# coreyjadams/SparseEventID

Measured on NVIDIA B200. Metric: 3D sparse ResNet train events/sec, higher is better.
Workload: dtype bf16

## Files before the change

sparseeventid_b200/csrc/conv_tc.cu:

```cuda
#include <cstdlib>
#include <cstring>

#include "common.cuh"
#include "tc_ptx.cuh"

namespace tc {

constexpr int BM = 128;
constexpr int KC = 64;
constexpr int KC_TF32 = 32;
constexpr int A_BYTES = BM * 128;
constexpr int EPI_WARPS = 4;
constexpr int NGRP = 4;
constexpr int PROD_WARPS = 4 * NGRP;
constexpr int WARP_MMA = EPI_WARPS + PROD_WARPS;
constexpr int MMA_WARPS = 4;
constexpr int WARP_BLOAD = WARP_MMA + MMA_WARPS;
constexpr int THREADS = 32 * (WARP_BLOAD + 1);
constexpr int MAX_A = 12, MAX_B = 8;
constexpr int MASK_BYTES = 32;
constexpr int LIST_BYTES = 64 * 8;
using namespace tcptx;

__device__ __forceinline__ uint64_t make_desc_sw128(uint32_t saddr) {
  uint64_t d = 0;
  d |= (uint64_t)((saddr & 0x3FFFFu) >> 4);
  d |= (uint64_t)1 << 16;
  d |= (uint64_t)(1024 >> 4) << 32;
  d |= (uint64_t)1 << 46;
  d |= (uint64_t)2 << 61;
  return d;
}
__device__ __forceinline__ const unsigned char* mad_wide16(uint32_t units, const unsigned char* base) {
  uint64_t r;
  asm("mad.wide.u32 %0, %1, 16, %2;" : "=l"(r) : "r"(units), "l"((uint64_t)(uintptr_t)base));
  return reinterpret_cast<const unsigned char*>((uintptr_t)r);
}
template <bool TF32>
__device__ __forceinline__ uint32_t make_idesc(int n) {
  constexpr uint32_t fmt = TF32 ? 2u : 1u;
  return (1u << 4) | (fmt << 7) | (fmt << 10) | ((uint32_t)(n >> 3) << 17) | ((uint32_t)(BM >> 4) << 24);
}
template <bool TF32>
__device__ __forceinline__ void store8(void* out, int64_t idx, const float* f) {
  if constexpr (TF32) {
    float4* d = reinterpret_cast<float4*>(reinterpret_cast<float*>(out) + idx);
    d[0] = make_float4(f[0], f[1], f[2], f[3]);
    d[1] = make_float4(f[4], f[5], f[6], f[7]);
  } else {
    uint4 u;
    u.x = pack_bf16x2(f[0], f[1]); u.y = pack_bf16x2(f[2], f[3]);
    u.z = pack_bf16x2(f[4], f[5]); u.w = pack_bf16x2(f[6], f[7]);
    *reinterpret_cast<uint4*>(reinterpret_cast<__nv_bfloat16*>(out) + idx) = u;
  }
}
struct Params {
  const void* in;
  const int32_t* nbr;
  const unsigned char* bimg;
  const float* bias;
  void* out;
  int64_t n_rows, n_pad;
  int K, n_in, n_out;
  int nch;
  int last_kc;
  int T;
  int SA, SB;
  int num_tiles;
  int NM;
  int nbuf;
  int ksplit;
  unsigned long long* dbg;
  int exp;
};

template <int NCH, bool PAIR, bool TF32 = false>
__global__ void __launch_bounds__(THREADS, 1) k_conv_tc(const Params p) {
  static_assert(!(TF32 && PAIR), "a 32-channel fp32 row fills a stage");
  constexpr int ESZ = TF32 ? 4 : 2;
  constexpr int KCE = 128 / ESZ;
  const int nch = NCH > 0 ? NCH : p.nch;
  extern __shared__ unsigned char smem_raw[];
  pdl_launch_dependents();
  const uint32_t raw = smem_u32(smem_raw);
  const uint32_t base = (raw + 1023u) & ~1023u;
  unsigned char* gbase = smem_raw + (base - raw);
  const int SA = p.SA, SB = p.SB;
  const uint32_t b_bytes = (uint32_t)p.n_out * 128u;
  const uint32_t a_base = base;
  const uint32_t b_base = base + (uint32_t)SA * A_BYTES;
  const uint32_t bar0 = b_base + (uint32_t)SB * b_bytes;
  auto afull = [&](int s) { return bar0 + 8u * (uint32_t)s; };
  auto aempty = [&](int s) { return bar0 + 8u * (uint32_t)(MAX_A + s); };
  auto bfull = [&](int s) { return bar0 + 8u * (uint32_t)(2 * MAX_A + s); };
  auto bempty = [&](int s) { return bar0 + 8u * (uint32_t)(2 * MAX_A + MAX_B + s); };
  auto accf = [&](int b) { return bar0 + 8u * (uint32_t)(2 * MAX_A + 2 * MAX_B + b); };
  auto acce = [&](int b) { return bar0 + 8u * (uint32_t)(2 * MAX_A + 2 * MAX_B + 2 + b); };
  constexpr int NBAR = 2 * MAX_A + 2 * MAX_B + 4;
  unsigned char* tail = gbase + (size_t)SA * A_BYTES + (size_t)SB * b_bytes + 8 * NBAR;
  uint32_t* tmem_slot = reinterpret_cast<uint32_t*>(tail);
  uint32_t* amask = reinterpret_cast<uint32_t*>(tail + 16);
  unsigned char* lists = tail + 16 + MAX_A * MASK_BYTES;

  const int warp = __shfl_sync(0xffffffffu, (int)(threadIdx.x >> 5), 0), lane = threadIdx.x & 31;
  auto mark = [&](int role, int stage, int ev) {
#ifdef SCN_TC_TIMELINE
    if (p.dbg != nullptr && blockIdx.x == 0 && lane == 0 && stage < 256)
      p.dbg[((size_t)role * 256 + stage) * 8 + ev] = (unsigned long long)clock64();
#else
    (void)role; (void)stage; (void)ev;
#endif
  };
#ifdef SCN_TC_TIMELINE
  const int exp_flags = p.exp;
#else
  constexpr int exp_flags = 0;
#endif

  const int T = p.T;
  const int tile_lo = (int)(((int64_t)p.num_tiles * blockIdx.x) / gridDim.x);
  const int tile_hi = (int)(((int64_t)p.num_tiles * (blockIdx.x + 1)) / gridDim.x);
  const int my_tiles = tile_hi - tile_lo;
  const int my_groups = (my_tiles + T - 1) / T;
  auto tiles_in_group = [&](int g) { return my_tiles - g * T < T ? my_tiles - g * T : T; };
  const int NSTEP = PAIR ? (p.K + 1) / 2 : p.K;
  const int Q = NSTEP * nch;
  const bool ksplit = p.ksplit != 0 && p.NM == 2 && my_tiles == 1;

  if (warp == WARP_MMA) {
    if (lane == 0) {
      for (int s = 0; s < SA; ++s) {
        mbar_init(afull(s), 132);
        mbar_init(aempty(s), 1);
      }
      for (int s = 0; s < SB; ++s) {
        mbar_init(bfull(s), 1);
        mbar_init(bempty(s), ksplit ? 1 : p.NM);
      }
      for (int b = 0; b < 2; ++b) {
        mbar_init(accf(b), p.NM);
        mbar_init(acce(b), EPI_WARPS);
      }
      asm volatile("fence.mbarrier_init.release.cluster;" ::: "memory");
    }
    __syncwarp();
    asm volatile("tcgen05.alloc.cta_group::1.sync.aligned.shared::cta.b32 [%0], %1;" ::"r"(smem_u32(tmem_slot)), "r"(512)
                 : "memory");
    asm volatile("tcgen05.relinquish_alloc_permit.cta_group::1.sync.aligned;" ::: "memory");
  }
  tc_fence_before();
  __syncthreads();
  tc_fence_after();
  const uint32_t tmem_base = *tmem_slot;
  pdl_wait();

  const int NM = p.NM;
  const int spc = SA / NM;

  if (warp >= EPI_WARPS && warp < EPI_WARPS + PROD_WARPS) {
    const int pw = warp - EPI_WARPS;
    const int grp = pw >> 2, wq = pw & 3;
    const int cls = grp % NM, sub = grp / NM, gpc = NGRP / NM;
    constexpr int LPI = PAIR ? 4 : 8;
    constexpr int IPP = 32 / LPI;
    const int chunk = lane % LPI, isub = lane / LPI;
    const uint32_t row_vec = (uint32_t)p.n_in >> (TF32 ? 2 : 3);
    const int last_chunks = p.last_kc * ESZ / 16;
    const uint32_t lt = (1u << lane) - 1u;
    const uint32_t csw = (uint32_t)chunk << 4;
    const uint32_t myrow = 32u * (uint32_t)wq + (uint32_t)lane;
    const uint32_t drow = a_base + (myrow << 7) + ((myrow & 7u) << 4);

    int t = cls, q = 0, cc = 0, g = 0, tv = my_groups > 0 ? tiles_in_group(0) : 0;
    const int32_t* gptr = p.nbr + (int64_t)tile_lo * BM + myrow;
    const int32_t* qptr = gptr;
    const int64_t qstride = (int64_t)p.n_pad * (PAIR ? 2 : 1);
    auto next_q = [&]() {
      ++q;
      if (++cc == nch) { cc = 0; qptr += qstride; }
    };
    auto step = [&]() {
      if (ksplit) {
        next_q(); next_q();
        if (q >= Q) { g = my_groups; tv = 0; }
        return;
      }
      t += NM;
      if (t >= tv) {
        t = cls;
        next_q();
        if (q == Q) {
          q = 0; ++g;
          gptr += (int64_t)T * BM;
          qptr = gptr;
          tv = g < my_groups ? tiles_in_group(g) : 0;
        }
      }
    };
    auto valid = [&]() { return g < my_groups && (ksplit ? q < Q : cls < tv); };
    if (ksplit) {
      t = 0;
      if (cls == 1) next_q();
    }
    for (int i = 0; i < sub; ++i)
      if (valid()) step();
    auto fetch = [&](int& jl_, int& jh_, int& q_) {
      q_ = -1; jl_ = -1; jh_ = -1;
      if (valid()) {
        const int32_t* src = qptr + t * BM;
        jl_ = ldg_nc32(src);
        if (PAIR && (2 * q + 1 < p.K)) jh_ = ldg_nc32(src + p.n_pad);
        q_ = (q << 3) | cc;
        for (int i = 0; i < gpc; ++i) step();
      }
    };

    int ls = sub;
    uint32_t round = 0;
    int it = 0;
    auto do_stage = [&](const int jl, const int jh, const int qc) {
      if (wq == 0) mark(grp, it, 0);
      int2* list = reinterpret_cast<int2*>(lists + (pw * 2 + (it & 1)) * LIST_BYTES);
      const int slot = cls * spc + ls;
      const int ccur = qc & 7;
      const bool full = qc < (ksplit ? 16 : 8);
      const uint32_t dst = drow + (uint32_t)slot * A_BYTES;
      const uint32_t bl = __ballot_sync(0xffffffffu, jl >= 0);
      const uint32_t bh = PAIR ? __ballot_sync(0xffffffffu, jh >= 0) : 0u;
      int nlive;
      if (full) {
        list[lane] = make_int2(jl >= 0 ? (int)((uint32_t)jl * row_vec) : -1, (int)dst);
        if (PAIR) list[32 + lane] = make_int2(jh >= 0 ? (int)((uint32_t)jh * row_vec) : -1, (int)(dst ^ 0x40u));
        nlive = PAIR ? 64 : 32;
      } else {
        const int2 el = make_int2((int)((uint32_t)jl * row_vec), (int)dst);
        const int2 eh = make_int2((int)((uint32_t)jh * row_vec), (int)(dst ^ 0x40u));
        if (jl >= 0) list[__popc(bl & lt)] = el;
        nlive = __popc(bl);
        if (PAIR) {
          if (jh >= 0) list[nlive + __popc(bh & lt)] = eh;
          nlive += __popc(bh);
        }
        if (nlive & (IPP - 1)) {
          const bool from_hi = PAIR && bh != 0u;
          const int top = 31 - __clz(from_hi ? bh : bl);
          const int lx = __shfl_sync(0xffffffffu, from_hi ? eh.x : el.x, top);
          const int ly = __shfl_sync(0xffffffffu, from_hi ? eh.y : el.y, top);
          const int padded = (nlive + IPP - 1) & ~(IPP - 1);
          if (nlive + lane < padded) list[nlive + lane] = make_int2(lx, ly);
        }
      }
      __syncwarp();
      if (wq == 0) mark(grp, it, 1);

      mbar_wait(aempty(slot), (round & 1u) ^ 1u);
      if (wq == 0) mark(grp, it, 2);
      if (lane == 0) {
        amask[slot * 8 + wq] = ~bl;
        if (PAIR) amask[slot * 8 + 4 + wq] = ~bh;
      }
      const int npass = (nlive + IPP - 1) / IPP;
      const bool lane_on = PAIR ? true : chunk < (ccur == nch - 1 ? last_chunks : 8);
      const unsigned char* src0 = reinterpret_cast<const unsigned char*>(p.in) + ((uint32_t)ccur * 128u + csw);
      if (lane_on && !(exp_flags & 1)) {
        if (!full) {
          for (int p0 = 0; p0 < npass; p0 += 4) {
            int2 e[4];
#pragma unroll
            for (int u = 0; u < 4; ++u)
              if (p0 + u < npass) e[u] = list[(p0 + u) * IPP + isub];
#pragma unroll
            for (int u = 0; u < 4; ++u)
              if (p0 + u < npass) cp_async16((uint32_t)e[u].y ^ csw, mad_wide16((uint32_t)e[u].x, src0), 16u);
          }
        } else {
#pragma unroll
          for (int pass = 0; pass < 8; ++pass) {
            const int2 e = list[pass * IPP + isub];
            const bool live = e.x != -1;
            cp_async16((uint32_t)e.y ^ csw, mad_wide16(live ? (uint32_t)e.x : 0u, src0), live ? 16u : 0u);
          }
        }
      }
      cp_async_arrive_noinc(afull(slot));
      if (lane == 0) mbar_arrive(afull(slot));
      if (wq == 0) mark(grp, it, 3);
      ++it;
      ls += gpc;
      if (ls >= spc) { ls -= spc; ++round; }
    };

    int jlA, jhA, qA, jlB, jhB, qB;
    fetch(jlA, jhA, qA);
    fetch(jlB, jhB, qB);
    while (qA >= 0) {
      int jlC, jhC, qC;
      fetch(jlC, jhC, qC);
      do_stage(jlA, jhA, qA);
      jlA = jlB; jhA = jhB; qA = qB;
      jlB = jlC; jhB = jhC; qB = qC;
    }
  } else if (warp == WARP_BLOAD) {
    const int total_b = my_groups * Q;
    int bslot = 0;
    uint32_t bround = 0;
    for (int i = 0; i < total_b; ++i) {
      mark(8, i, 0);
      if (ksplit) mbar_wait_sleep(bempty(bslot), (bround & 1u) ^ 1u, 100u);
      else mbar_wait(bempty(bslot), (bround & 1u) ^ 1u);
      mark(8, i, 1);
      if (elect_one()) {
        mbar_expect_tx(bfull(bslot), b_bytes);
        bulk_g2s(b_base + (uint32_t)bslot * b_bytes, p.bimg + (size_t)(i % Q) * b_bytes, b_bytes, bfull(bslot));
      }
      __syncwarp();
      if (++bslot == SB) { bslot = 0; ++bround; }
    }
  } else if (warp >= WARP_MMA && warp < WARP_MMA + MMA_WARPS) {
    const int m = warp - WARP_MMA;
    if (m < NM) {
      const uint32_t idesc = make_idesc<TF32>(p.n_out);
      const uint64_t da0 = make_desc_sw128(a_base), db0 = make_desc_sw128(b_base);
      const int nbuf = p.nbuf;
      int bslot = 0;
      uint32_t bround = 0;
      int ls = 0;
      uint32_t around = 0;
      int it = 0;
      auto issue_stage = [&](int q, uint32_t col, uint64_t db, bool first) {
        const int cc = PAIR ? 0 : q % nch;
        const int step = PAIR ? q : q / nch;
        const int nk = PAIR ? ((2 * step + 1 < p.K) ? 4 : 2) : ((cc == nch - 1 ? p.last_kc : KCE) * ESZ / 32);
        const int aslot = m * spc + ls;
        mark(4 + m, it, 0);
        mbar_wait(afull(aslot), around & 1u);
        mark(4 + m, it, 1);
        tc_fence_after();
        uint32_t m0 = 0, m1 = 0, m2 = 0, m3 = 0, h0 = 0, h1 = 0, h2 = 0, h3 = 0;
        if (!first) {
          const uint4 mw = *reinterpret_cast<const uint4*>(amask + aslot * 8);
          m0 = __ballot_sync(0xffffffffu, (mw.x >> lane) & 1u);
          m1 = __ballot_sync(0xffffffffu, (mw.y >> lane) & 1u);
          m2 = __ballot_sync(0xffffffffu, (mw.z >> lane) & 1u);
          m3 = __ballot_sync(0xffffffffu, (mw.w >> lane) & 1u);
          if (PAIR) {
            const uint4 hw = *reinterpret_cast<const uint4*>(amask + aslot * 8 + 4);
            h0 = __ballot_sync(0xffffffffu, (hw.x >> lane) & 1u);
            h1 = __ballot_sync(0xffffffffu, (hw.y >> lane) & 1u);
            h2 = __ballot_sync(0xffffffffu, (hw.z >> lane) & 1u);
            h3 = __ballot_sync(0xffffffffu, (hw.w >> lane) & 1u);
          }
        }
        const uint64_t da = da0 + (uint64_t)((uint32_t)aslot * (A_BYTES >> 4));
        const uint32_t tmem_d = tmem_base + col;
        if (elect_one()) {
#pragma unroll
          for (int kk = 0; kk < 4; ++kk) {
            if (kk < nk && !(exp_flags & 2)) {
              const bool hi = PAIR && kk >= 2;
              umma_masked<TF32>(tmem_d, da + (uint64_t)(kk * 2), db + (uint64_t)(kk * 2), idesc, (!first || kk > 0) ? 1u : 0u,
                                hi ? h0 : m0, hi ? h1 : m1, hi ? h2 : m2, hi ? h3 : m3);
            }
          }
          umma_commit(aempty(aslot));
        }
        __syncwarp();
        mark(4 + m, it, 2);
        ++it;
        if (++ls == spc) { ls = 0; ++around; }
      };
      if (ksplit) {
        mbar_wait(acce(0), 1u);
        tc_fence_after();
        bslot = m;
        for (int q = m; q < Q; q += 2) {
          mbar_wait(bfull(bslot), bround & 1u);
          issue_stage(q, (uint32_t)(m * p.n_out), db0 + (uint64_t)(((uint32_t)bslot * b_bytes) >> 4), q < 2);
          if (elect_one()) umma_commit(bempty(bslot));
          __syncwarp();
          bslot += 2;
          if (bslot >= SB) { bslot -= SB; ++bround; }
        }
        if (elect_one()) umma_commit(accf(0));
        __syncwarp();
      } else
      for (int g = 0; g < my_groups; ++g) {
        const int buf = nbuf == 2 ? (g & 1) : 0;
        const uint32_t use = (uint32_t)(nbuf == 2 ? (g >> 1) : g);
        const int tv = tiles_in_group(g);
        mbar_wait(acce(buf), (use & 1u) ^ 1u);
        tc_fence_after();
        for (int q = 0; q < Q; ++q) {
          mark(10 + m, g * Q + q, 0);
          mbar_wait(bfull(bslot), bround & 1u);
          mark(10 + m, g * Q + q, 1);
          const uint64_t db = db0 + (uint64_t)(((uint32_t)bslot * b_bytes) >> 4);
          for (int t = m; t < tv; t += NM) issue_stage(q, (uint32_t)buf * 256u + (uint32_t)(t * p.n_out), db, q == 0);
          if (elect_one()) umma_commit(bempty(bslot));
          __syncwarp();
          if (++bslot == SB) { bslot = 0; ++bround; }
        }
        if (elect_one()) umma_commit(accf(buf));
        __syncwarp();
      }
    }
  } else if (warp < EPI_WARPS) {
    if (ksplit) {
      mbar_wait_sleep(accf(0), 0u, 100u);
      tc_fence_after();
      const int64_t row = (int64_t)tile_lo * BM + warp * 32 + lane;
      const uint32_t taddr = tmem_base + ((uint32_t)(warp * 32) << 16);
      for (int c0 = 0; c0 < p.n_out; c0 += 16) {
        uint32_t a[16], b[16];
        tmem_ld16x2(taddr + (uint32_t)c0, taddr + (uint32_t)(p.n_out + c0), a, b);
        if (row < p.n_rows && !(exp_flags & 4)) {
#pragma unroll
          for (int gq = 0; gq < 2; ++gq) {
            float f[8];
#pragma unroll
            for (int e = 0; e < 8; ++e)
              f[e] = __uint_as_float(a[gq * 8 + e]) + __uint_as_float(b[gq * 8 + e]) +
                     (p.bias ? __ldg(p.bias + c0 + gq * 8 + e) : 0.f);
            store8<TF32>(p.out, row * p.n_out + c0 + gq * 8, f);
          }
        }
      }
      tc_fence_before();
    } else
    for (int g = 0; g < my_groups; ++g) {
      const int buf = p.nbuf == 2 ? (g & 1) : 0;
      if (warp == 0) mark(9, g, 0);
      mbar_wait_long(accf(buf), (uint32_t)(p.nbuf == 2 ? (g >> 1) : g) & 1u);
      if (warp == 0) mark(9, g, 1);
      tc_fence_after();
      const int tv = tiles_in_group(g);
      for (int t = 0; t < tv; ++t) {
        const int64_t tile = (int64_t)tile_lo + (int64_t)g * T + t;
        const int64_t row = tile * BM + warp * 32 + lane;
        const uint32_t taddr = tmem_base + ((uint32_t)(warp * 32) << 16) + (uint32_t)buf * 256u + (uint32_t)(t * p.n_out);
        for (int c0 = 0; c0 < p.n_out; c0 += 32) {
          uint32_t v[32];
          tmem_ld32(taddr + (uint32_t)c0, v);
          if (row < p.n_rows && !(exp_flags & 4)) {
#pragma unroll
            for (int gq = 0; gq < 4; ++gq) {
              float f[8];
#pragma unroll
              for (int e = 0; e < 8; ++e)
                f[e] = __uint_as_float(v[gq * 8 + e]) + (p.bias ? __ldg(p.bias + c0 + gq * 8 + e) : 0.f);
              store8<TF32>(p.out, row * p.n_out + c0 + gq * 8, f);
            }
          }
        }
      }
      tc_fence_before();
      __syncwarp();
      if (warp == 0) mark(9, g, 2);
      if (lane == 0) mbar_arrive(acce(buf));
    }
  }

  tc_fence_before();
  __syncthreads();
  if (warp == WARP_MMA) {
    tc_fence_after();
    asm volatile("tcgen05.dealloc.cta_group::1.sync.aligned.b32 %0, %1;" ::"r"(tmem_base), "r"(512) : "memory");
  }
}

__global__ void k_prep_weights_tc(const float* __restrict__ W, int K, int Cin, int Cout, int transpose, int mirror,
                                  int nch, int pair, int tf32, void* __restrict__ img) {
  const int n_in = transpose ? Cout : Cin, n_out = transpose ? Cin : Cout;
  int64_t total = (int64_t)K * n_in * n_out;
  int64_t i = blockIdx.x * (int64_t)blockDim.x + threadIdx.x;
  if (i >= total) return;
  int k = (int)(i / ((int64_t)n_in * n_out));
  int rem = (int)(i - (int64_t)k * n_in * n_out);
  int n = rem / n_in, c = rem % n_in;
  int src_k = (transpose && mirror) ? K - 1 - k : k;
  int ci = transpose ? n : c, co = transpose ? c : n;
  float v = W[((int64_t)src_k * Cin + ci) * Cout + co];
  if (tf32) {
    const int q = k * nch + c / KC_TF32, chunk = (c % KC_TF32) >> 2;
    reinterpret_cast<float*>(img)[((size_t)q * n_out + n) * 32 + (size_t)((chunk ^ (n & 7)) << 2) + (c & 3)] = to_tf32_rna(v);
    return;
  }
  const int q = pair ? (k >> 1) : k * nch + c / KC;
  const int chunk = pair ? (k & 1) * 4 + (c >> 3) : (c % KC) >> 3;
  size_t off = ((size_t)q * n_out + n) * 64 + (size_t)((chunk ^ (n & 7)) << 3) + (c & 7);
  reinterpret_cast<__nv_bfloat16*>(img)[off] = __float2bfloat16_rn(v);
}

__global__ void __launch_bounds__(256) k_prep_weights_tc_batched(const long long* __restrict__ descs, int n, long long units) {
  pdl_launch_dependents();
  pdl_wait();
  const long long i = blockIdx.x * (long long)blockDim.x + threadIdx.x;
  if (i >= units) return;
  const long long e = i * 8;
  int lo = 0, hi = n - 1;
  while (lo < hi) {
    const int mid = (lo + hi + 1) >> 1;
    if (__ldg(descs + mid * 8 + 6) <= e) lo = mid; else hi = mid - 1;
  }
  const long long* d = descs + lo * 8;
  const float* W = reinterpret_cast<const float*>(d[0]);
  unsigned char* img = reinterpret_cast<unsigned char*>(d[1]);
  const int K = (int)d[2], Cin = (int)d[3], Cout = (int)d[4], transpose = (int)(d[5] & 1), mirror = (int)((d[5] >> 1) & 1);
  const int n_in = transpose ? Cout : Cin, n_out = transpose ? Cin : Cout;
  const bool tf32 = d[7] == SCN_PREC_TF32;
  const int kc = tf32 ? KC_TF32 : KC;
  const int nch = (n_in + kc - 1) / kc, pair = !tf32 && n_in == 32;
  const int u = (int)((e - d[6]) >> 3);
  const int per_k = (n_in >> 3) * n_out;
  const int k = u / per_k;
  const int r = u - k * per_k;
  const int cb = r / n_out, nn = r - cb * n_out;
  const int c0 = cb * 8;
  const int src_k = (transpose && mirror) ? K - 1 - k : k;
  float v[8];
  if (transpose) {
    const float4* src = reinterpret_cast<const float4*>(W + ((long long)src_k * Cin + nn) * Cout + c0);
    const float4 a = __ldg(src), b = __ldg(src + 1);
    v[0] = a.x; v[1] = a.y; v[2] = a.z; v[3] = a.w; v[4] = b.x; v[5] = b.y; v[6] = b.z; v[7] = b.w;
  } else {
    const float* src = W + ((long long)src_k * Cin + c0) * Cout + nn;
#pragma unroll
    for (int j = 0; j < 8; ++j) v[j] = __ldg(src + (long long)j * Cout);
  }
  if (tf32) {
    const int q = k * nch + c0 / KC_TF32, chunk = (c0 % KC_TF32) >> 2;
    unsigned char* row = img + ((size_t)q * n_out + nn) * 128;
    *reinterpret_cast<float4*>(row + ((chunk ^ (nn & 7)) << 4)) =
        make_float4(to_tf32_rna(v[0]), to_tf32_rna(v[1]), to_tf32_rna(v[2]), to_tf32_rna(v[3]));
    *reinterpret_cast<float4*>(row + (((chunk + 1) ^ (nn & 7)) << 4)) =
        make_float4(to_tf32_rna(v[4]), to_tf32_rna(v[5]), to_tf32_rna(v[6]), to_tf32_rna(v[7]));
    return;
  }
  const int q = pair ? (k >> 1) : k * nch + c0 / KC;
  const int chunk = pair ? (k & 1) * 4 + cb : (c0 % KC) >> 3;
  uint4 o;
  o.x = pack_bf16x2(v[0], v[1]); o.y = pack_bf16x2(v[2], v[3]);
  o.z = pack_bf16x2(v[4], v[5]); o.w = pack_bf16x2(v[6], v[7]);
  *reinterpret_cast<uint4*>(img + ((size_t)q * n_out + nn) * 128 + (size_t)((chunk ^ (nn & 7)) << 4)) = o;
}

}

extern "C" int scn_conv_prep_weights_batched(const void* descs, int n, int64_t total, void* stream) {
  if (n <= 0 || total <= 0) return SCN_OK;
  if (!descs) return SCN_ERR_ARG;
  SCN_CUDA(scn_launch_pdl(tc::k_prep_weights_tc_batched, dim3(grid_for(total / 8, 256)), dim3(256), 0, (cudaStream_t)stream,
                          (const long long*)descs, n, (long long)(total / 8)));
  SCN_LAUNCH_CHECK();
  return SCN_OK;
}

static unsigned long long* g_tc_dbg = nullptr;
extern "C" void scn_tc_debug_timeline(void* device_buffer) { g_tc_dbg = (unsigned long long*)device_buffer; }
#ifdef SCN_TC_TIMELINE
static int g_tc_exp = 0;
extern "C" void scn_tc_debug_exp(int flags) { g_tc_exp = flags; }
#else
extern "C" void scn_tc_debug_exp(int) {}
#endif

bool scn_tc_disabled() {
  static int v = -1;
  if (v < 0) {
    const char* e = std::getenv("SCN_B200_DISABLE_TC");
    v = (e && e[0] && e[0] != '0') ? 1 : 0;
  }
  return v == 1;
}

bool scn_tc_shape_ok(int K, int n_in, int n_out) {
  return K >= 1 && (n_in % 32) == 0 && (n_out % 32) == 0 && n_in >= 32 && n_in <= 256 && n_out >= 32 && n_out <= 256;
}

static bool tc_pair(int n_in, int tf32) { return !tf32 && n_in == 32; }
static int tc_nch(int n_in, int tf32) {
  const int kc = tf32 ? tc::KC_TF32 : tc::KC;
  return (n_in + kc - 1) / kc;
}

size_t scn_tc_image_bytes(int K, int n_in, int n_out, int tf32) {
  const size_t stages = tc_pair(n_in, tf32) ? (size_t)(K + 1) / 2 : (size_t)K * tc_nch(n_in, tf32);
  return stages * n_out * 128;
}

int scn_tc_prep(const float* W, int K, int Cin, int Cout, int transpose, int mirror, int tf32, void* out, cudaStream_t s) {
  const int n_in = transpose ? Cout : Cin, n_out = transpose ? Cin : Cout;
  const int nch = tc_nch(n_in, tf32);
  if (!tf32 && (n_in % tc::KC) != 0) SCN_CUDA(cudaMemsetAsync(out, 0, scn_tc_image_bytes(K, n_in, n_out, tf32), s));
  int64_t total = (int64_t)K * Cin * Cout;
  tc::k_prep_weights_tc<<<grid_for(total, 256), 256, 0, s>>>(W, K, Cin, Cout, transpose, mirror, nch,
                                                             tc_pair(n_in, tf32) ? 1 : 0, tf32, out);
  SCN_LAUNCH_CHECK();
  return SCN_OK;
}

static int env_int(const char* name) {
  const char* e = std::getenv(name);
  return e ? std::atoi(e) : 0;
}
static bool g_ksplit_enabled() {
  static int v = -1;
  if (v < 0) {
    const char* e = std::getenv("SCN_B200_TC_KSPLIT");
    v = (e && e[0] == '0') ? 0 : 1;
  }
  return v == 1;
}
static int g_knob[4] = {-1, -1, -1, -1};
extern "C" void scn_tc_debug_knobs(int grid, int t, int sa, int sb) {
  g_knob[0] = grid; g_knob[1] = t; g_knob[2] = sa; g_knob[3] = sb;
}
static int32_t g_last_launch[9] = {0, 0, 0, 0, 0, 0, 0, 0, 0};
extern "C" void scn_tc_debug_last_launch(int32_t* out) {
  for (int i = 0; i < 9; ++i) out[i] = g_last_launch[i];
}

int scn_tc_forward(const void* in, int64_t n_in_rows, const int32_t* nbr, int K, int64_t n_rows, int64_t n_pad, int n_in,
                   int n_out, const void* bimg, const float* bias, void* out, int tf32, cudaStream_t s) {
  const uint64_t row_units = (uint64_t)n_in * (tf32 ? 4u : 2u) / 16u;
  if ((uint64_t)n_in_rows * row_units >= 0xffffffffull) return SCN_ERR_UNSUPPORTED;
  if (g_knob[0] < 0) {
    g_knob[0] = env_int("SCN_B200_TC_GRID"); g_knob[1] = env_int("SCN_B200_TC_T");
    g_knob[2] = env_int("SCN_B200_TC_SA"); g_knob[3] = env_int("SCN_B200_TC_SB");
  }
  const int force_grid = g_knob[0], force_t = g_knob[1], force_sa = g_knob[2], force_sb = g_knob[3];
  tc::Params p;
  p.dbg = g_tc_dbg;
#ifdef SCN_TC_TIMELINE
  p.exp = g_tc_exp;
#else
  p.exp = 0;
#endif
  p.in = in; p.nbr = nbr; p.bimg = (const unsigned char*)bimg; p.bias = bias; p.out = out;
  p.n_rows = n_rows; p.n_pad = n_pad; p.K = K; p.n_in = n_in; p.n_out = n_out;
  const bool pair = tc_pair(n_in, tf32);
  const int nch = tc_nch(n_in, tf32);
  p.nch = nch;
  p.last_kc = n_in - (nch - 1) * (tf32 ? tc::KC_TF32 : tc::KC);
  p.num_tiles = (int)((n_rows + tc::BM - 1) / tc::BM);
  int max_ctas = kNumSMs;
  if (force_grid > 0 && force_grid < max_ctas) max_ctas = force_grid;
  const int per_cta = (p.num_tiles + max_ctas - 1) / max_ctas;
  const int q_per_tile = (pair ? (K + 1) / 2 : K) * nch;
  int T = 1;
  p.nbuf = 2;
  {
    double best = 1e30;
    for (int t = 1; t <= 8 && t * n_out <= 512 && t <= (per_cta > 0 ? per_cta : 1); ++t) {
      const int nm = t >= 4 ? 4 : (t >= 2 ? 2 : 1);
      const int full = per_cta / t, rem = per_cta % t;
      const int groups = full + (rem ? 1 : 0);
      const double units = (double)full * ((t + nm - 1) / nm) + (rem ? (rem + nm - 1) / nm : 0);
      const int nbuf = t * n_out <= 256 ? 2 : 1;
      const double ep = (double)t * (n_out / 32.0) * 600.0 / ((double)q_per_tile * 1400.0);
      const double cost = units + (nbuf == 1 ? groups * ep : ep + 0.15 * (groups - 1) * ep);
      if (cost <= best + 1e-9) { best = cost; T = t; p.nbuf = nbuf; }
    }
  }
  if (force_t > 0) {
    T = force_t;
    if (T > 8) T = 8;
    if (T * n_out > 512) T = 512 / n_out;
    if (T > per_cta) T = per_cta;
    if (T < 1) T = 1;
    p.nbuf = T * n_out <= 256 ? 2 : 1;
  }
  p.T = T;
  p.NM = T >= 4 ? 4 : (T >= 2 ? 2 : 1);
  p.ksplit = 0;
  const int stages_per_tile = (pair ? (K + 1) / 2 : K) * nch;
  if (g_ksplit_enabled() && stages_per_tile >= 2) {
    if (p.NM == 1 && per_cta == 1 && 2 * n_out <= 512) { p.NM = 2; p.nbuf = 1; p.ksplit = 1; }
    else if (p.NM == 2) p.ksplit = 1;
  }
  const uint32_t b_bytes = (uint32_t)n_out * 128u;
  constexpr int NBAR = 2 * tc::MAX_A + 2 * tc::MAX_B + 4;
  const uint32_t fixed = 1024u + 8u * NBAR + 16u + (uint32_t)tc::MAX_A * tc::MASK_BYTES +
                         2u * (uint32_t)tc::PROD_WARPS * tc::LIST_BYTES + 16u;
  const uint32_t budget = 226u * 1024u - fixed;
  int SA = 8;
  if (p.ksplit && per_cta <= 2) SA = 4;
  if (force_sa > 0) SA = force_sa;
  SA = SA / tc::NGRP * tc::NGRP;
  if (SA > tc::MAX_A) SA = tc::MAX_A;
  if (SA < tc::NGRP) SA = tc::NGRP;
  while (SA > tc::NGRP && (uint32_t)SA * tc::A_BYTES + 2u * b_bytes > budget) SA -= tc::NGRP;
  if ((uint32_t)SA * tc::A_BYTES + 2u * b_bytes > budget) return SCN_ERR_UNSUPPORTED;
  int SB = (int)((budget - (uint32_t)SA * tc::A_BYTES) / b_bytes);
  if (SB > tc::MAX_B) SB = tc::MAX_B;
  if (force_sb >= 2 && force_sb < SB) SB = force_sb;
  if (p.ksplit && (SB & 1)) --SB;
  p.SA = SA;
  p.SB = SB;
  const size_t smem = (size_t)fixed + (size_t)SA * tc::A_BYTES + (size_t)SB * b_bytes;
  int grid = p.num_tiles < max_ctas ? p.num_tiles : max_ctas;
  {
    static bool attr_set = false;
    if (!attr_set) {
      SCN_CUDA(cudaFuncSetAttribute(tc::k_conv_tc<1, true>, cudaFuncAttributeMaxDynamicSharedMemorySize, 227 * 1024));
      SCN_CUDA(cudaFuncSetAttribute(tc::k_conv_tc<1, false>, cudaFuncAttributeMaxDynamicSharedMemorySize, 227 * 1024));
      SCN_CUDA(cudaFuncSetAttribute(tc::k_conv_tc<2, false>, cudaFuncAttributeMaxDynamicSharedMemorySize, 227 * 1024));
      SCN_CUDA(cudaFuncSetAttribute(tc::k_conv_tc<3, false>, cudaFuncAttributeMaxDynamicSharedMemorySize, 227 * 1024));
      SCN_CUDA(cudaFuncSetAttribute(tc::k_conv_tc<4, false>, cudaFuncAttributeMaxDynamicSharedMemorySize, 227 * 1024));
      SCN_CUDA(cudaFuncSetAttribute(tc::k_conv_tc<0, false, true>, cudaFuncAttributeMaxDynamicSharedMemorySize, 227 * 1024));
      attr_set = true;
    }
  }
  if (grid < 1) return SCN_OK;
  {
    const int32_t rec[9] = {grid, p.T, p.NM, p.nbuf, p.ksplit, p.SA, p.SB, p.num_tiles / grid,
                            (p.num_tiles + grid - 1) / grid};
    for (int i = 0; i < 9; ++i) g_last_launch[i] = rec[i];
  }
  auto launch = [&](auto kern) -> int {
    SCN_CUDA(scn_launch_pdl(kern, dim3((unsigned)grid), dim3(tc::THREADS), smem, s, p));
    SCN_LAUNCH_CHECK();
    return SCN_OK;
  };
  if (tf32) return nch <= 8 ? launch(tc::k_conv_tc<0, false, true>) : SCN_ERR_UNSUPPORTED;
  if (pair) return launch(tc::k_conv_tc<1, true>);
  switch (nch) {
    case 1: return launch(tc::k_conv_tc<1, false>);
    case 2: return launch(tc::k_conv_tc<2, false>);
    case 3: return launch(tc::k_conv_tc<3, false>);
    case 4: return launch(tc::k_conv_tc<4, false>);
    default: return SCN_ERR_UNSUPPORTED;
  }
}
```

Before: 3563.

## Generalize K-split into stream-K style stage partitioning with fp32 partial fixup

Replaces the old K-split, which only applied to single-tile CTAs with two MMA halves, with a stream-K scheme. The flattened tile×stage space is divided evenly across CTAs, and each CTA processes pieces of possibly several tiles. Tiles split across CTAs write fp32 partials to a global workspace, and the last arriving CTA (tracked with an atomic counter) reduces them and adds bias. The aim is better SM load balance when there are few tiles or uneven tile counts, at the cost of extra global traffic for partials, atomics and fixup work. The grid can grow to num_tiles*Q/8 CTAs.

Result: slower. 3351, median of 6 (-6.0%).

```diff
diff --git a/sparseeventid_b200/csrc/conv_tc.cu b/sparseeventid_b200/csrc/conv_tc.cu
--- a/sparseeventid_b200/csrc/conv_tc.cu
+++ b/sparseeventid_b200/csrc/conv_tc.cu
@@ -1,5 +1,7 @@
 #include <cstdlib>
 #include <cstring>
+#include <map>
+#include <mutex>
 
 #include "common.cuh"
 #include "tc_ptx.cuh"
@@ -54,6 +56,7 @@
     *reinterpret_cast<uint4*>(reinterpret_cast<__nv_bfloat16*>(out) + idx) = u;
   }
 }
+__device__ __forceinline__ void epi_bar_sync() { asm volatile("bar.sync 1, %0;" ::"n"(EPI_WARPS * 32) : "memory"); }
 struct Params {
   const void* in;
   const int32_t* nbr;
@@ -70,6 +73,9 @@
   int NM;
   int nbuf;
   int ksplit;
+  float* part;
+  int* cnt;
+  int maxc;
   unsigned long long* dbg;
   int exp;
 };
@@ -101,6 +107,8 @@
   uint32_t* tmem_slot = reinterpret_cast<uint32_t*>(tail);
   uint32_t* amask = reinterpret_cast<uint32_t*>(tail + 16);
   unsigned char* lists = tail + 16 + MAX_A * MASK_BYTES;
+  volatile int* final_tile = reinterpret_cast<volatile int*>(tmem_slot + 2);
+  if (threadIdx.x == 0) *final_tile = -1;
 
   const int warp = __shfl_sync(0xffffffffu, (int)(threadIdx.x >> 5), 0), lane = threadIdx.x & 31;
   auto mark = [&](int role, int stage, int ev) {
@@ -125,7 +133,44 @@
   auto tiles_in_group = [&](int g) { return my_tiles - g * T < T ? my_tiles - g * T : T; };
   const int NSTEP = PAIR ? (p.K + 1) / 2 : p.K;
   const int Q = NSTEP * nch;
-  const bool ksplit = p.ksplit != 0 && p.NM == 2 && my_tiles == 1;
+  const bool split = p.ksplit != 0;
+  const int S = split ? p.num_tiles * Q : 0;
+  const int s0 = (int)(((int64_t)S * blockIdx.x) / gridDim.x), s1 = (int)(((int64_t)S * (blockIdx.x + 1)) / gridDim.x);
+  const int t0 = split ? s0 / Q : 0;
+  const int npieces = s1 > s0 ? (s1 - 1) / Q - t0 + 1 : 0;
+  auto piece = [&](int k, int& tile, int& qa, int& qe) {
+    tile = t0 + k;
+    qa = k == 0 ? s0 - t0 * Q : 0;
+    qe = s1 - tile * Q < Q ? s1 - tile * Q : Q;
+  };
+  auto owner = [&](int s) { return (int)(((int64_t)(s + 1) * gridDim.x - 1) / S); };
+  auto fixup = [&](int tile, int tid, int nthreads) {
+    const int n_out = p.n_out, lo = owner(tile * Q), nc = owner(tile * Q + Q - 1) - lo + 1;
+    const float4* base = reinterpret_cast<const float4*>(p.part + (size_t)tile * p.maxc * BM * n_out);
+    const size_t slot4 = (size_t)BM * n_out / 4;
+    for (int idx = tid; idx < BM * (n_out >> 3); idx += nthreads) {
+      const int r = idx & (BM - 1), c8 = idx / BM;
+      const int64_t row = (int64_t)tile * BM + r;
+      if (row >= p.n_rows || (exp_flags & 4)) continue;
+      const float4* src = base + (size_t)(2 * c8) * BM + r;
+      float f[8];
+      for (int j0 = 0; j0 < nc; j0 += 2) {
+        const float4 a0 = __ldcg(src + j0 * slot4), a1 = __ldcg(src + j0 * slot4 + BM);
+        float4 b0 = make_float4(0.f, 0.f, 0.f, 0.f), b1 = b0;
+        if (j0 + 1 < nc) { b0 = __ldcg(src + (j0 + 1) * slot4); b1 = __ldcg(src + (j0 + 1) * slot4 + BM); }
+        const float va[8] = {a0.x, a0.y, a0.z, a0.w, a1.x, a1.y, a1.z, a1.w};
+        const float vb[8] = {b0.x, b0.y, b0.z, b0.w, b1.x, b1.y, b1.z, b1.w};
+#pragma unroll
+        for (int e = 0; e < 8; ++e) {
+          f[e] = j0 == 0 ? va[e] : f[e] + va[e];
+          if (j0 + 1 < nc) f[e] += vb[e];
+        }
+      }
+#pragma unroll
+      for (int e = 0; e < 8; ++e) f[e] += p.bias ? __ldg(p.bias + c8 * 8 + e) : 0.f;
+      store8<TF32>(p.out, row * n_out + c8 * 8, f);
+    }
+  };
 
   if (warp == WARP_MMA) {
     if (lane == 0) {
@@ -135,7 +180,7 @@
       }
       for (int s = 0; s < SB; ++s) {
         mbar_init(bfull(s), 1);
-        mbar_init(bempty(s), ksplit ? 1 : p.NM);
+        mbar_init(bempty(s), split ? 1 : p.NM);
       }
       for (int b = 0; b < 2; ++b) {
         mbar_init(accf(b), p.NM);
@@ -175,14 +220,27 @@
     const int32_t* gptr = p.nbr + (int64_t)tile_lo * BM + myrow;
     const int32_t* qptr = gptr;
     const int64_t qstride = (int64_t)p.n_pad * (PAIR ? 2 : 1);
+    int qa = 0, qe = Q;
     auto next_q = [&]() {
       ++q;
       if (++cc == nch) { cc = 0; qptr += qstride; }
     };
+    auto enter_piece = [&]() {
+      for (; g < npieces; ++g) {
+        int tile;
+        piece(g, tile, qa, qe);
+        q = qa + cls;
+        if (q < qe) {
+          cc = q % nch;
+          qptr = p.nbr + (int64_t)tile * BM + myrow + (int64_t)(q / nch) * qstride;
+          return;
+        }
+      }
+    };
     auto step = [&]() {
-      if (ksplit) {
+      if (split) {
         next_q(); next_q();
-        if (q >= Q) { g = my_groups; tv = 0; }
+        if (q >= qe) { ++g; enter_piece(); }
         return;
       }
       t += NM;
@@ -197,10 +255,10 @@
         }
       }
     };
-    auto valid = [&]() { return g < my_groups && (ksplit ? q < Q : cls < tv); };
-    if (ksplit) {
+    auto valid = [&]() { return split ? g < npieces : g < my_groups && cls < tv; };
+    if (split) {
       t = 0;
-      if (cls == 1) next_q();
+      enter_piece();
     }
     for (int i = 0; i < sub; ++i)
       if (valid()) step();
@@ -210,7 +268,7 @@
         const int32_t* src = qptr + t * BM;
         jl_ = ldg_nc32(src);
         if (PAIR && (2 * q + 1 < p.K)) jh_ = ldg_nc32(src + p.n_pad);
-        q_ = (q << 3) | cc;
+        q_ = (q << 4) | ((split ? q < qa + 2 : q == 0) ? 8 : 0) | cc;
         for (int i = 0; i < gpc; ++i) step();
       }
     };
@@ -223,7 +281,7 @@
       int2* list = reinterpret_cast<int2*>(lists + (pw * 2 + (it & 1)) * LIST_BYTES);
       const int slot = cls * spc + ls;
       const int ccur = qc & 7;
-      const bool full = qc < (ksplit ? 16 : 8);
+      const bool full = (qc & 8) != 0;
       const uint32_t dst = drow + (uint32_t)slot * A_BYTES;
       const uint32_t bl = __ballot_sync(0xffffffffu, jl >= 0);
       const uint32_t bh = PAIR ? __ballot_sync(0xffffffffu, jh >= 0) : 0u;
@@ -301,13 +359,32 @@
       jlB = jlC; jhB = jhC; qB = qC;
     }
   } else if (warp == WARP_BLOAD) {
-    const int total_b = my_groups * Q;
+    if (split) {
+      int bs0 = 0, bs1 = 1;
+      uint32_t br0 = 0, br1 = 0;
+      for (int k = 0; k < npieces; ++k) {
+        int tile, qa, qe;
+        piece(k, tile, qa, qe);
+        for (int q = qa; q < qe; ++q) {
+          const bool c1 = ((q - qa) & 1) != 0;
+          const int bslot = c1 ? bs1 : bs0;
+          mbar_wait_sleep(bempty(bslot), ((c1 ? br1 : br0) & 1u) ^ 1u, 100u);
+          if (elect_one()) {
+            mbar_expect_tx(bfull(bslot), b_bytes);
+            bulk_g2s(b_base + (uint32_t)bslot * b_bytes, p.bimg + (size_t)q * b_bytes, b_bytes, bfull(bslot));
+          }
+          __syncwarp();
+          if (c1) { if ((bs1 += 2) >= SB) { bs1 -= SB; ++br1; } }
+          else    { if ((bs0 += 2) >= SB) { bs0 -= SB; ++br0; } }
+        }
+      }
+    }
+    const int total_b = split ? 0 : my_groups * Q;
     int bslot = 0;
     uint32_t bround = 0;
     for (int i = 0; i < total_b; ++i) {
       mark(8, i, 0);
-      if (ksplit) mbar_wait_sleep(bempty(bslot), (bround & 1u) ^ 1u, 100u);
-      else mbar_wait(bempty(bslot), (bround & 1u) ^ 1u);
+      mbar_wait(bempty(bslot), (bround & 1u) ^ 1u);
       mark(8, i, 1);
       if (elect_one()) {
         mbar_expect_tx(bfull(bslot), b_bytes);
@@ -369,20 +446,24 @@
         ++it;
         if (++ls == spc) { ls = 0; ++around; }
       };
-      if (ksplit) {
-        mbar_wait(acce(0), 1u);
-        tc_fence_after();
+      if (split) {
         bslot = m;
-        for (int q = m; q < Q; q += 2) {
-          mbar_wait(bfull(bslot), bround & 1u);
-          issue_stage(q, (uint32_t)(m * p.n_out), db0 + (uint64_t)(((uint32_t)bslot * b_bytes) >> 4), q < 2);
-          if (elect_one()) umma_commit(bempty(bslot));
+        for (int k = 0; k < npieces; ++k) {
+          int tile, qa, qe;
+          piece(k, tile, qa, qe);
+          mbar_wait(acce(0), (k & 1) ^ 1u);
+          tc_fence_after();
+          for (int q = qa + m; q < qe; q += 2) {
+            mbar_wait(bfull(bslot), bround & 1u);
+            issue_stage(q, (uint32_t)(m * p.n_out), db0 + (uint64_t)(((uint32_t)bslot * b_bytes) >> 4), q < qa + 2);
+            if (elect_one()) umma_commit(bempty(bslot));
+            __syncwarp();
+            bslot += 2;
+            if (bslot >= SB) { bslot -= SB; ++bround; }
+          }
+          if (elect_one()) umma_commit(accf(0));
           __syncwarp();
-          bslot += 2;
-          if (bslot >= SB) { bslot -= SB; ++bround; }
-        }
-        if (elect_one()) umma_commit(accf(0));
-        __syncwarp();
+        }
       } else
       for (int g = 0; g < my_groups; ++g) {
         const int buf = nbuf == 2 ? (g & 1) : 0;
@@ -405,27 +486,60 @@
       }
     }
   } else if (warp < EPI_WARPS) {
-    if (ksplit) {
-      mbar_wait_sleep(accf(0), 0u, 100u);
-      tc_fence_after();
-      const int64_t row = (int64_t)tile_lo * BM + warp * 32 + lane;
+    if (split) {
+      volatile int* last_flag = reinterpret_cast<volatile int*>(tmem_slot + 1);
       const uint32_t taddr = tmem_base + ((uint32_t)(warp * 32) << 16);
-      for (int c0 = 0; c0 < p.n_out; c0 += 16) {
-        uint32_t a[16], b[16];
-        tmem_ld16x2(taddr + (uint32_t)c0, taddr + (uint32_t)(p.n_out + c0), a, b);
-        if (row < p.n_rows && !(exp_flags & 4)) {
-#pragma unroll
-          for (int gq = 0; gq < 2; ++gq) {
-            float f[8];
-#pragma unroll
-            for (int e = 0; e < 8; ++e)
-              f[e] = __uint_as_float(a[gq * 8 + e]) + __uint_as_float(b[gq * 8 + e]) +
-                     (p.bias ? __ldg(p.bias + c0 + gq * 8 + e) : 0.f);
-            store8<TF32>(p.out, row * p.n_out + c0 + gq * 8, f);
+      const int n_out = p.n_out;
+      const int r = warp * 32 + lane;
+      for (int k = 0; k < npieces; ++k) {
+        int tile, qa, qe;
+        piece(k, tile, qa, qe);
+        const int lo = owner(tile * Q), nc = owner(tile * Q + Q - 1) - lo + 1;
+        const bool two = qe - qa >= 2;
+        const int64_t row = (int64_t)tile * BM + r;
+        const bool live = row < p.n_rows && !(exp_flags & 4);
+        float4* slot = reinterpret_cast<float4*>(p.part + (size_t)(tile * p.maxc + (int)blockIdx.x - lo) * BM * n_out) + r;
+        mbar_wait_sleep(accf(0), (uint32_t)k & 1u, 100u);
+        tc_fence_after();
+        for (int c0 = 0; c0 < n_out; c0 += 16) {
+          uint32_t a[16], b[16];
+          tmem_ld16x2(taddr + (uint32_t)c0, taddr + (uint32_t)(n_out + c0), a, b);
+          if (live) {
+#pragma unroll
+            for (int gq = 0; gq < 2; ++gq) {
+              float f[8];
+#pragma unroll
+              for (int e = 0; e < 8; ++e)
+                f[e] = two ? __uint_as_float(a[gq * 8 + e]) + __uint_as_float(b[gq * 8 + e]) : __uint_as_float(a[gq * 8 + e]);
+              if (nc == 1) {
+#pragma unroll
+                for (int e = 0; e < 8; ++e) f[e] += p.bias ? __ldg(p.bias + c0 + gq * 8 + e) : 0.f;
+                store8<TF32>(p.out, row * n_out + c0 + gq * 8, f);
+              } else {
+                float4* d = slot + (size_t)((c0 + gq * 8) >> 2) * BM;
+                d[0] = make_float4(f[0], f[1], f[2], f[3]);
+                d[BM] = make_float4(f[4], f[5], f[6], f[7]);
+              }
+            }
           }
         }
-      }
-      tc_fence_before();
+        tc_fence_before();
+        __syncwarp();
+        if (lane == 0) mbar_arrive(acce(0));
+        if (nc == 1) continue;
+        __threadfence();
+        epi_bar_sync();
+        if (warp == 0 && lane == 0) {
+          const int prev = atomicAdd(p.cnt + tile, 1);
+          const int last = prev == nc - 1;
+          if (last) p.cnt[tile] = 0;
+          __threadfence();
+          if (last && k + 1 == npieces) *final_tile = tile;
+          *last_flag = last && k + 1 < npieces;
+        }
+        epi_bar_sync();
+        if (*last_flag) fixup(tile, (int)threadIdx.x, EPI_WARPS * 32);
+      }
     } else
     for (int g = 0; g < my_groups; ++g) {
       const int buf = p.nbuf == 2 ? (g & 1) : 0;
@@ -462,6 +576,7 @@
 
   tc_fence_before();
   __syncthreads();
+  if (split && *final_tile >= 0) fixup(*final_tile, (int)threadIdx.x, THREADS);
   if (warp == WARP_MMA) {
     tc_fence_after();
     asm volatile("tcgen05.dealloc.cta_group::1.sync.aligned.b32 %0, %1;" ::"r"(tmem_base), "r"(512) : "memory");
@@ -611,6 +726,7 @@
   }
   return v == 1;
 }
+static constexpr int kSplitMinStages = 8;
 static int g_knob[4] = {-1, -1, -1, -1};
 extern "C" void scn_tc_debug_knobs(int grid, int t, int sa, int sb) {
   g_knob[0] = grid; g_knob[1] = t; g_knob[2] = sa; g_knob[3] = sb;
@@ -618,6 +734,41 @@
 static int32_t g_last_launch[9] = {0, 0, 0, 0, 0, 0, 0, 0, 0};
 extern "C" void scn_tc_debug_last_launch(int32_t* out) {
   for (int i = 0; i < 9; ++i) out[i] = g_last_launch[i];
+}
+static int32_t g_last_split[6] = {0, 0, 0, 0, 0, 0};
+extern "C" void scn_tc_debug_last_split(int32_t* out) {
+  for (int i = 0; i < 6; ++i) out[i] = g_last_split[i];
+}
+
+namespace {
+struct SplitWs { float* part = nullptr; size_t part_bytes = 0; int* cnt = nullptr; size_t n_cnt = 0; };
+int split_workspace(size_t part_bytes, size_t n_cnt, cudaStream_t s, float** part, int** cnt) {
+  static std::mutex mu;
+  static std::map<std::pair<int, cudaStream_t>, SplitWs> table;
+  int dev = 0;
+  SCN_CUDA(cudaGetDevice(&dev));
+  std::lock_guard<std::mutex> lock(mu);
+  SplitWs& w = table[{dev, s}];
+  if (w.part_bytes < part_bytes || w.n_cnt < n_cnt) {
+    SCN_CUDA(cudaStreamSynchronize(s));
+    if (w.part_bytes < part_bytes) {
+      cudaFree(w.part);
+      w.part = nullptr; w.part_bytes = 0;
+      SCN_CUDA(cudaMalloc(&w.part, part_bytes + part_bytes / 4));
+      w.part_bytes = part_bytes + part_bytes / 4;
+    }
+    if (w.n_cnt < n_cnt) {
+      cudaFree(w.cnt);
+      w.cnt = nullptr; w.n_cnt = 0;
+      SCN_CUDA(cudaMalloc(&w.cnt, n_cnt * sizeof(int)));
+      SCN_CUDA(cudaMemsetAsync(w.cnt, 0, n_cnt * sizeof(int), s));
+      w.n_cnt = n_cnt;
+    }
+  }
+  *part = w.part;
+  *cnt = w.cnt;
+  return SCN_OK;
+}
 }
 
 int scn_tc_forward(const void* in, int64_t n_in_rows, const int32_t* nbr, int K, int64_t n_rows, int64_t n_pad, int n_in,
@@ -673,18 +824,14 @@
   p.T = T;
   p.NM = T >= 4 ? 4 : (T >= 2 ? 2 : 1);
   p.ksplit = 0;
-  const int stages_per_tile = (pair ? (K + 1) / 2 : K) * nch;
-  if (g_ksplit_enabled() && stages_per_tile >= 2) {
-    if (p.NM == 1 && per_cta == 1 && 2 * n_out <= 512) { p.NM = 2; p.nbuf = 1; p.ksplit = 1; }
-    else if (p.NM == 2) p.ksplit = 1;
-  }
+  if (g_ksplit_enabled() && q_per_tile >= 2 && per_cta <= 2) { p.NM = 2; p.nbuf = 1; p.ksplit = 1; }
   const uint32_t b_bytes = (uint32_t)n_out * 128u;
   constexpr int NBAR = 2 * tc::MAX_A + 2 * tc::MAX_B + 4;
   const uint32_t fixed = 1024u + 8u * NBAR + 16u + (uint32_t)tc::MAX_A * tc::MASK_BYTES +
                          2u * (uint32_t)tc::PROD_WARPS * tc::LIST_BYTES + 16u;
   const uint32_t budget = 226u * 1024u - fixed;
   int SA = 8;
-  if (p.ksplit && per_cta <= 2) SA = 4;
+  if (p.ksplit) SA = 4;
   if (force_sa > 0) SA = force_sa;
   SA = SA / tc::NGRP * tc::NGRP;
   if (SA > tc::MAX_A) SA = tc::MAX_A;
@@ -699,6 +846,41 @@
   p.SB = SB;
   const size_t smem = (size_t)fixed + (size_t)SA * tc::A_BYTES + (size_t)SB * b_bytes;
   int grid = p.num_tiles < max_ctas ? p.num_tiles : max_ctas;
+  p.part = nullptr; p.cnt = nullptr; p.maxc = 1;
+  for (int i = 0; i < 6; ++i) g_last_split[i] = 0;
+  if (p.ksplit && grid >= 1) {
+    const int S = p.num_tiles * q_per_tile;
+    if (force_grid > 0) grid = max_ctas < S ? max_ctas : S;
+    else if (S / kSplitMinStages > grid) grid = S / kSplitMinStages < max_ctas ? S / kSplitMinStages : max_ctas;
+    auto owner = [&](int st) { return (int)(((int64_t)(st + 1) * grid - 1) / S); };
+    int fixups = 0, maxc = 1;
+    for (int t = 0; t < p.num_tiles; ++t) {
+      const int nc = owner(t * q_per_tile + q_per_tile - 1) - owner(t * q_per_tile) + 1;
+      if (nc > 1) ++fixups;
+      if (nc > maxc) maxc = nc;
+    }
+    int max_stages = 0, max_pieces = 0, min_piece = q_per_tile, odd = 0;
+    for (int b = 0; b < grid; ++b) {
+      const int s0 = (int)((int64_t)S * b / grid), s1 = (int)((int64_t)S * (b + 1) / grid);
+      if (s1 - s0 > max_stages) max_stages = s1 - s0;
+      const int np = (s1 - 1) / q_per_tile - s0 / q_per_tile + 1;
+      if (np > max_pieces) max_pieces = np;
+      for (int t = s0 / q_per_tile; t * q_per_tile < s1; ++t) {
+        const int a = s0 > t * q_per_tile ? s0 : t * q_per_tile;
+        const int e = s1 < (t + 1) * q_per_tile ? s1 : (t + 1) * q_per_tile;
+        if (e - a < min_piece) min_piece = e - a;
+        odd += (e - a) & 1;
+      }
+    }
+    const int32_t rec[6] = {max_stages, max_pieces, min_piece, odd, fixups, maxc};
+    for (int i = 0; i < 6; ++i) g_last_split[i] = rec[i];
+    p.maxc = maxc;
+    if (maxc > 1) {
+      const int r = split_workspace((size_t)p.num_tiles * maxc * tc::BM * n_out * sizeof(float), (size_t)p.num_tiles, s,
+                                    &p.part, &p.cnt);
+      if (r != SCN_OK) return r;
+    }
+  }
   {
     static bool attr_set = false;
     if (!attr_set) {
```
